# Bob-cheng/DepthModelHardening

Measured on AMD Instinct MI355X. Metric: adv-train images/sec @1024x320, 10-step PGD, bs32, higher is better.
Workload: dtype f32; 1 GPU; Monodepth2 ResNet18 1024x320, 10-step PGD-L_inf attack on 12 scenes, train batch 32/GPU, stereo photometric+SSIM+smoothness loss (md2), Adam; config_index=2, global_batch=32, per_gpu_batch=32, parallelism=dp1, attack_overlap=False, attack_scenes=12, graph_attack=False

## Files before the change

### depthmodelhardening_amd/csrc/stem_conv_fwd.hip

```cpp
#include "common.hpp"

using namespace dmh;

namespace {

typedef float f32x16 __attribute__((ext_vector_type(16)));

constexpr int NT = 256;
constexpr int TR = 4, TC = 32;
constexpr int RH = 2 * TR + 5;
constexpr int RW = 2 * TC + 6;
constexpr int PLANE = RH * RW;
constexpr int NPAIR = 74;

struct PairDesc { int off; int cls; int k0; int k1; };
__host__ __device__ constexpr PairDesc pair_desc(int j) {
    if (j < 63) {
        const int c = j / 21, r = j % 21, ky = r / 3, kx = 2 * (r % 3);
        return {c * PLANE + ky * RW + kx, 0, c * 49 + ky * 7 + kx, c * 49 + ky * 7 + kx + 1};
    }
    if (j < 72) {
        const int q = j - 63, c = q / 3, ky = 2 * (q % 3);
        return {c * PLANE + ky * RW + 6, 1, c * 49 + ky * 7 + 6, c * 49 + (ky + 1) * 7 + 6};
    }
    if (j == 72) return {6 * RW + 6, 2, 0 * 49 + 48, 1 * 49 + 48};
    return {2 * PLANE + 6 * RW + 6, 0, 2 * 49 + 48, -1};
}

struct SArgs {
    const float* x;
    const float* w;
    float* y;
    int B, H, W, Ho, Wo, gx, gy, ntiles;
    float mean, inv_std;
    const int* org;
    int hw, ww;
};

__global__ __launch_bounds__(NT, 2) void stem_conv_fwd_kernel(const SArgs a) {
    __shared__ float tile[3 * PLANE];
    const int tid = threadIdx.x, lane = tid & 63, wv = tid >> 6;
    const int n = lane & 31, h = lane >> 5;

    float wA[NPAIR], wB[NPAIR];
#pragma unroll
    for (int j = 0; j < NPAIR; ++j) {
        const PairDesc d = pair_desc(j);
        const int kk = h ? d.k1 : d.k0;
        wA[j] = kk >= 0 ? a.w[(size_t)n * 147 + kk] : 0.f;
        wB[j] = kk >= 0 ? a.w[(size_t)(n + 32) * 147 + kk] : 0.f;
    }
    const int base = (2 * wv) * RW + 2 * n;
    const float* b0 = tile + base + (h ? 1 : 0);
    const float* b1 = tile + base + (h ? RW : 0);
    const float* b2 = tile + base + (h ? PLANE : 0);

    const size_t HW = (size_t)a.H * a.W, HWo = (size_t)a.hw * a.ww;
    for (int t = blockIdx.x; t < a.ntiles; t += gridDim.x) {
        int q = t;
        const int bxi = q % a.gx;  q /= a.gx;
        const int byi = q % a.gy;
        const int b = q / a.gy;
        const int wy0 = a.org ? a.org[2 * b] : 0, wx0 = a.org ? a.org[2 * b + 1] : 0;
        const int oy0 = wy0 + byi * TR, ox0 = wx0 + bxi * TC;
        const int iy0 = 2 * oy0 - 3, ix0 = 2 * ox0 - 3;
        const float* xb = a.x + (size_t)b * 3 * HW;
        __syncthreads();
        for (int e = tid; e < 3 * PLANE; e += NT) {
            const int c = e / PLANE, rem = e - c * PLANE, r = rem / RW, cc = rem - r * RW;
            const int iy = iy0 + r, ix = ix0 + cc;
            const bool ok = iy >= 0 && iy < a.H && ix >= 0 && ix < a.W;
            const float v = xb[(size_t)c * HW + (size_t)min(max(iy, 0), a.H - 1) * a.W + min(max(ix, 0), a.W - 1)];
            tile[e] = ok ? (v - a.mean) * a.inv_std : 0.f;
        }
        __syncthreads();
        f32x16 accA, accB;
#pragma unroll
        for (int v = 0; v < 16; ++v) accA[v] = accB[v] = 0.f;
#pragma unroll
        for (int j = 0; j < NPAIR; ++j) {
            const PairDesc d = pair_desc(j);
            const float bv = (d.cls == 0 ? b0 : d.cls == 1 ? b1 : b2)[d.off];
            accA = __builtin_amdgcn_mfma_f32_32x32x2f32(wA[j], bv, accA, 0, 0, 0);
            accB = __builtin_amdgcn_mfma_f32_32x32x2f32(wB[j], bv, accB, 0, 0, 0);
        }
        const int oy = oy0 + wv - wy0, ox = ox0 + n - wx0;
        if (oy < a.hw && ox < a.ww) {
            float* yb = a.y + (size_t)b * 64 * HWo + (size_t)oy * a.ww + ox;
#pragma unroll
            for (int v = 0; v < 16; ++v) {
                const int i = 8 * (v >> 2) + 4 * h + (v & 3);
                yb[(size_t)i * HWo] = accA[v];
                yb[(size_t)(i + 32) * HWo] = accB[v];
            }
        }
    }
}

inline long long stem_fwd_tiles(int B, int hw, int ww) {
    return (long long)B * ((ww + TC - 1) / TC) * ((hw + TR - 1) / TR);
}
inline int stem_fwd_workgroups(long long tiles) { return (int)(tiles < 512 ? tiles : 512); }

}

extern "C" {

static int launch_stem_fwd(const float* x, const float* w, const int* org, int B, int H, int W, int hw, int ww, float mean,
                           float std, float* y, void* stream, const char* fn) {
    SArgs a;
    a.x = x;
    a.w = w;
    a.y = y;
    a.B = B;
    a.H = H;
    a.W = W;
    a.Ho = H / 2;
    a.Wo = W / 2;
    a.org = org;
    a.hw = hw;
    a.ww = ww;
    a.gx = (ww + TC - 1) / TC;
    a.gy = (hw + TR - 1) / TR;
    const long long tiles = stem_fwd_tiles(B, hw, ww);
    if (tiles >= (1ll << 31)) return fail(DMH_EINVAL, "%s: grid too large", fn);
    a.ntiles = (int)tiles;
    a.mean = mean;
    a.inv_std = 1.0f / std;
    const int blocks = stem_fwd_workgroups(tiles);
    hipLaunchKernelGGL(stem_conv_fwd_kernel, dim3(blocks), dim3(NT), 0, (hipStream_t)stream, a);
    return check_launch(fn);
}

int dmh_stem_conv_norm_fwd(const float* x, const float* w, int B, int H, int W, float mean, float std, float* y,
                           void* stream) {
    DMH_REQUIRE(x && w && y, "null pointer");
    DMH_REQUIRE(B > 0 && H >= 2 && W >= 2 && (H & 1) == 0 && (W & 1) == 0, "image height and width must be even");
    DMH_REQUIRE(std > 0.f, "std must be positive");
    DMH_REQUIRE((int64_t)B * 64 * (H / 2) * (W / 2) < ((int64_t)1 << 40), "tensor too large");
    return launch_stem_fwd(x, w, nullptr, B, H, W, H / 2, W / 2, mean, std, y, stream, "dmh_stem_conv_norm_fwd");
}

int64_t dmh_stem_conv_norm_fwd_tiles(int B, int H, int W) {
    if (B <= 0 || H < 2 || W < 2 || (H & 1) || (W & 1)) return -1;
    return stem_fwd_tiles(B, H / 2, W / 2);
}

int dmh_stem_conv_norm_fwd_workgroups(int B, int H, int W) {
    const int64_t tiles = dmh_stem_conv_norm_fwd_tiles(B, H, W);
    return tiles < 0 || tiles >= ((int64_t)1 << 31) ? -1 : stem_fwd_workgroups(tiles);
}

int dmh_stem_conv_norm_fwd_win(const float* x, const float* w, const int* org, int B, int H, int W, int hw, int ww, float mean,
                               float std, float* y, void* stream) {
    DMH_REQUIRE(x && w && y && org, "null pointer");
    DMH_REQUIRE(B > 0 && H >= 2 && W >= 2 && (H & 1) == 0 && (W & 1) == 0, "image height and width must be even");
    DMH_REQUIRE(std > 0.f, "std must be positive");
    DMH_REQUIRE(hw >= 1 && ww >= 1 && hw <= H / 2 && ww <= W / 2, "the window must lie inside the H/2 x W/2 output");
    return launch_stem_fwd(x, w, org, B, H, W, hw, ww, mean, std, y, stream, "dmh_stem_conv_norm_fwd_win");
}

}
```

Baseline: 408.7 images/s.

## Stage stem filters in LDS and load input tile with 128-bit buffer loads

The kernel now copies the full 64x147 filter bank into shared memory with vectorized buffer loads, and each lane gathers its MFMA operands from LDS instead of doing scattered global reads. The input tile fill switches from per-element clamped scalar loads to 16-byte aligned buffer loads with out-of-bounds masking. To allow this, the row width is padded to a multiple of 4 and a column offset is applied. The output store hoists the per-half channel offset and keeps the stride in a scalar register. The cost is extra LDS (about 37 KB for the filters) that may limit occupancy, plus a new 32-bit offset limit per image.

```diff
diff --git a/depthmodelhardening_amd/csrc/stem_conv_fwd.hip b/depthmodelhardening_amd/csrc/stem_conv_fwd.hip
--- a/depthmodelhardening_amd/csrc/stem_conv_fwd.hip
+++ b/depthmodelhardening_amd/csrc/stem_conv_fwd.hip
@@ -5,13 +5,20 @@
 namespace {
 
 typedef float f32x16 __attribute__((ext_vector_type(16)));
+typedef float f32x4 __attribute__((ext_vector_type(4)));
+
+#ifndef DMH_STEM_ABLATE
+#define DMH_STEM_ABLATE 0
+#endif
 
 constexpr int NT = 256;
 constexpr int TR = 4, TC = 32;
 constexpr int RH = 2 * TR + 5;
-constexpr int RW = 2 * TC + 6;
+constexpr int NWR = 18;
+constexpr int RW = 4 * NWR;
 constexpr int PLANE = RH * RW;
 constexpr int NPAIR = 74;
+constexpr int NFILT = 64 * 147;
 
 struct PairDesc { int off; int cls; int k0; int k1; };
 __host__ __device__ constexpr PairDesc pair_desc(int j) {
@@ -38,24 +45,41 @@
 };
 
 __global__ __launch_bounds__(NT, 2) void stem_conv_fwd_kernel(const SArgs a) {
-    __shared__ float tile[3 * PLANE];
+    __shared__ __attribute__((aligned(16))) float tile[3 * PLANE + 4];
     const int tid = threadIdx.x, lane = tid & 63, wv = tid >> 6;
     const int n = lane & 31, h = lane >> 5;
 
     float wA[NPAIR], wB[NPAIR];
+    __shared__ __attribute__((aligned(16))) float filt[NFILT];
+    {
+        constexpr int NWORD = NFILT / 4, PER_T = (NWORD + NT - 1) / NT;
+        const rsrc_t wrs = make_rsrc(a.w, (unsigned)NFILT * 4u);
+        f32x4 stage[PER_T];
+#pragma unroll
+        for (int k = 0; k < PER_T; ++k)
+            stage[k] = __builtin_bit_cast(f32x4, __builtin_amdgcn_raw_buffer_load_b128(wrs, (unsigned)(tid + NT * k) * 16u, 0, 0));
+#pragma unroll
+        for (int k = 0; k < PER_T; ++k)
+            if (tid + NT * k < NWORD) *reinterpret_cast<f32x4*>(filt + 4 * (tid + NT * k)) = stage[k];
+        if (tid < 4) tile[3 * PLANE + tid] = 0.f;
+        __syncthreads();
+    }
 #pragma unroll
     for (int j = 0; j < NPAIR; ++j) {
         const PairDesc d = pair_desc(j);
         const int kk = h ? d.k1 : d.k0;
-        wA[j] = kk >= 0 ? a.w[(size_t)n * 147 + kk] : 0.f;
-        wB[j] = kk >= 0 ? a.w[(size_t)(n + 32) * 147 + kk] : 0.f;
-    }
+        wA[j] = kk >= 0 ? filt[n * 147 + kk] : 0.f;
+        wB[j] = kk >= 0 ? filt[(n + 32) * 147 + kk] : 0.f;
+    }
+#if DMH_STEM_ABLATE & 1
+#pragma unroll
+    for (int j = 0; j < NPAIR; ++j) asm volatile("" ::"v"(wA[j]), "v"(wB[j]));
+    return;
+#endif
     const int base = (2 * wv) * RW + 2 * n;
-    const float* b0 = tile + base + (h ? 1 : 0);
-    const float* b1 = tile + base + (h ? RW : 0);
-    const float* b2 = tile + base + (h ? PLANE : 0);
 
     const size_t HW = (size_t)a.H * a.W, HWo = (size_t)a.hw * a.ww;
+    const size_t hoff = (size_t)(4 * h) * HWo;
     for (int t = blockIdx.x; t < a.ntiles; t += gridDim.x) {
         int q = t;
         const int bxi = q % a.gx;  q /= a.gx;
@@ -65,14 +89,28 @@
         const int oy0 = wy0 + byi * TR, ox0 = wx0 + bxi * TC;
         const int iy0 = 2 * oy0 - 3, ix0 = 2 * ox0 - 3;
         const float* xb = a.x + (size_t)b * 3 * HW;
+        const int coff = ix0 & 3, ixa = ix0 - coff;
+        const rsrc_t xrs = make_rsrc(xb, (unsigned)(3 * HW) * 4u);
+        constexpr int NITEM = 3 * RH * NWR, PER_S = (NITEM + NT - 1) / NT;
+        f32x4 stage[PER_S];
+#pragma unroll
+        for (int k = 0; k < PER_S; ++k) {
+            const int item = tid + NT * k, c = item / (RH * NWR), rem2 = item - c * (RH * NWR), r = rem2 / NWR, f = rem2 - r * NWR;
+            const int iy = iy0 + r, cx = ixa + 4 * f;
+            const bool ok = item < NITEM && iy >= 0 && iy < a.H && cx >= 0 && cx < a.W;
+            const unsigned vo = ok ? (unsigned)((c * a.H + iy) * a.W + cx) * 4u : 0xFFFFFFFFu;
+            f32x4 v = __builtin_bit_cast(f32x4, __builtin_amdgcn_raw_buffer_load_b128(xrs, vo, 0, 0));
+#pragma unroll
+            for (int e = 0; e < 4; ++e) v[e] = (ok && cx + e < a.W) ? (v[e] - a.mean) * a.inv_std : 0.f;
+            stage[k] = v;
+        }
         __syncthreads();
-        for (int e = tid; e < 3 * PLANE; e += NT) {
-            const int c = e / PLANE, rem = e - c * PLANE, r = rem / RW, cc = rem - r * RW;
-            const int iy = iy0 + r, ix = ix0 + cc;
-            const bool ok = iy >= 0 && iy < a.H && ix >= 0 && ix < a.W;
-            const float v = xb[(size_t)c * HW + (size_t)min(max(iy, 0), a.H - 1) * a.W + min(max(ix, 0), a.W - 1)];
-            tile[e] = ok ? (v - a.mean) * a.inv_std : 0.f;
-        }
+#pragma unroll
+        for (int k = 0; k < PER_S; ++k)
+            if (tid + NT * k < NITEM) *reinterpret_cast<f32x4*>(tile + 4 * (tid + NT * k)) = stage[k];
+        const float* b0 = tile + base + coff + (h ? 1 : 0);
+        const float* b1 = tile + base + coff + (h ? RW : 0);
+        const float* b2 = tile + base + coff + (h ? PLANE : 0);
         __syncthreads();
         f32x16 accA, accB;
 #pragma unroll
@@ -86,12 +124,14 @@
         }
         const int oy = oy0 + wv - wy0, ox = ox0 + n - wx0;
         if (oy < a.hw && ox < a.ww) {
-            float* yb = a.y + (size_t)b * 64 * HWo + (size_t)oy * a.ww + ox;
+            float* yb = a.y + (size_t)b * 64 * HWo + (size_t)oy * a.ww + ox + hoff;
+            size_t cs = HWo;
+            asm volatile("" : "+s"(cs));
 #pragma unroll
             for (int v = 0; v < 16; ++v) {
-                const int i = 8 * (v >> 2) + 4 * h + (v & 3);
-                yb[(size_t)i * HWo] = accA[v];
-                yb[(size_t)(i + 32) * HWo] = accB[v];
+                const int i = 8 * (v >> 2) + (v & 3);
+                yb[(size_t)i * cs] = accA[v];
+                yb[(size_t)(i + 32) * cs] = accB[v];
             }
         }
     }
@@ -138,6 +178,7 @@
     DMH_REQUIRE(B > 0 && H >= 2 && W >= 2 && (H & 1) == 0 && (W & 1) == 0, "image height and width must be even");
     DMH_REQUIRE(std > 0.f, "std must be positive");
     DMH_REQUIRE((int64_t)B * 64 * (H / 2) * (W / 2) < ((int64_t)1 << 40), "tensor too large");
+    DMH_REQUIRE((int64_t)H * W * 12 < ((int64_t)1 << 32), "one image must stay below 4 GiB (32-bit offsets per sample)");
     return launch_stem_fwd(x, w, nullptr, B, H, W, H / 2, W / 2, mean, std, y, stream, "dmh_stem_conv_norm_fwd");
 }
 
@@ -157,6 +198,7 @@
     DMH_REQUIRE(B > 0 && H >= 2 && W >= 2 && (H & 1) == 0 && (W & 1) == 0, "image height and width must be even");
     DMH_REQUIRE(std > 0.f, "std must be positive");
     DMH_REQUIRE(hw >= 1 && ww >= 1 && hw <= H / 2 && ww <= W / 2, "the window must lie inside the H/2 x W/2 output");
+    DMH_REQUIRE((int64_t)H * W * 12 < ((int64_t)1 << 32), "one image must stay below 4 GiB (32-bit offsets per sample)");
     return launch_stem_fwd(x, w, org, B, H, W, hw, ww, mean, std, y, stream, "dmh_stem_conv_norm_fwd_win");
 }
 
```

After: 410.9 images/s, median of 6. No clear change (+0.5%).
